# SeekStorm/SeekStorm

Measured on AMD Instinct MI355X. Metric: queries/sec (BM25 3-term OR top-10), higher is better.
Workload: dtype f32 sums of 16-bit posting weight codes (BM25); f32 MFMA (vector); 1 GPU; C2: 10M synthetic docs, 3-term OR BM25 top-10, one shard per GPU; host pointers in, answers on the host; queries_per_call=1000, k=10

## Files before the change

### seekstorm_amd/csrc/bm25_probe.hip

```cpp
#include <cstdlib>
#include <type_traits>

#include "bm25_probe_body.h"


__global__ void __launch_bounds__(256) bm_partmax_kernel(const bm_vquery* __restrict__ qs, const float* __restrict__ submax, uint32_t n_sub,
                                                         uint32_t n_terms, uint32_t nq, uint32_t P, float* __restrict__ pmax) {
  const uint32_t a = (blockIdx.x * blockDim.x + threadIdx.x) >> 6;
  const int lane = threadIdx.x & 63;
  if (a >= nq * P) return;
  const uint32_t qi = a % nq, part = a / nq;
  const bm_vquery* __restrict__ Q = qs + qi;
  const uint32_t s_begin = (uint32_t)(((u64)n_sub * part) / P), s_end = (uint32_t)(((u64)n_sub * (part + 1)) / P);
  for (uint32_t t = 0; t < 4u; t++) {
    const uint32_t term = t < Q->n_terms ? Q->term[t] : n_terms;
    float m = 0.f;
    for (uint32_t sb = s_begin + (uint32_t)lane; sb < s_end; sb += 64u) m = fmaxf(m, submax[(size_t)term * n_sub + sb]);
#pragma unroll
    for (int o = 32; o > 0; o >>= 1) m = fmaxf(m, __shfl_xor(m, o));
    if (lane == 0) pmax[((size_t)qi * P + part) * 4u + t] = m;
  }
}

__global__ void __launch_bounds__(256) bm_qbound_kernel(const bm_vquery* __restrict__ qs, const float* __restrict__ submax, uint32_t n_sub,
                                                        uint32_t nq, float* __restrict__ qbound) {
  const uint32_t q = blockIdx.y, sb = blockIdx.x * blockDim.x + threadIdx.x;
  if (q >= nq || sb >= n_sub) return;
  const bm_vquery* __restrict__ Q = qs + q;
  float b = 0.f;
  for (uint32_t t = 0; t < Q->n_terms; t++) b = fmaf(Q->idf[t], submax[(size_t)Q->term[t] * n_sub + sb], b);
  qbound[(size_t)q * n_sub + sb] = b * 1.00001f;
}

constexpr int PB_STAGED_G = 4;
#ifndef PB_STAGED_WAVES
#define PB_STAGED_WAVES 2
#endif
#ifndef PB_STAGED_MIN_WAVES
#define PB_STAGED_MIN_WAVES 6
#endif
static_assert(PB_STAGED_WAVES == 1 || PB_STAGED_WAVES == 2 || PB_STAGED_WAVES == 4 || PB_STAGED_WAVES == 8, "PB_STAGED_WAVES");
static_assert(PB_STAGED_MIN_WAVES == 6 || PB_STAGED_MIN_WAVES == 8, "PB_STAGED_MIN_WAVES");
static_assert((32 / PB_STAGED_WAVES) * (PB_STAGED_WAVES * pb_wave_lds(4, PB_STAGED_G)) <= 160 * 1024,
              "8 waves per SIMD of the staged kernel (32 / PB_STAGED_WAVES workgroups) must fit a CU's LDS");
constexpr int pb_staged_min_waves(int NT, int KPL, bool FILT, bool SKIP, bool HIST) {
  return KPL == 1 && !(NT == 4 && !FILT && !SKIP && HIST) ? PB_STAGED_MIN_WAVES : 6;
}
template <int NT, int KPL, bool FILT, bool SKIP, bool HIST>
__global__ void __launch_bounds__(PB_STAGED_WAVES * 64, pb_staged_min_waves(NT, KPL, FILT, SKIP, HIST)) bm25_probe_kernel(
    const uint32_t* __restrict__ post, const unsigned long long* __restrict__ term_base, const uint32_t* __restrict__ sub_off,
    const uint2* __restrict__ probe, const uint32_t* __restrict__ probe_z,
    const uint32_t* __restrict__ probe_row, const float* __restrict__ umax, const float* __restrict__ pmax, const float* __restrict__ qbound,
    const bm_vquery* __restrict__ qs, unsigned long long* __restrict__ part_keys, unsigned long long* __restrict__ total,
    uint32_t* tau, uint32_t* hist, const uint32_t* __restrict__ del, uint32_t del_words, uint32_t n_sub, uint32_t n_terms,
    uint32_t nq, uint32_t P, uint32_t k, uint32_t count) {
  extern __shared__ __attribute__((aligned(16))) char smem[];
  if ((uint32_t)(uintptr_t)(__attribute__((address_space(3))) char*)smem != 0u) __builtin_trap();
  const int tid = threadIdx.x, lane = tid & 63;
  const int w = __builtin_amdgcn_readfirstlane(tid >> 6);

  const uint32_t a = blockIdx.x * PB_STAGED_WAVES + w;
  if (a >= nq * P) return;
  const uint32_t qi = a % nq, part = a / nq;
  const BmTop<KPL> T = pb_wave<NT, KPL, FILT, SKIP, false, PB_STAGED_G, false, false, HIST>(
      post, term_base, sub_off, probe, probe_z, probe_row, umax, pmax, qbound, PbQueryMem{qs + qi}, tau, del, del_words, n_sub, n_terms, P, k, count, qi, part,
      w, lane, 0.f, nullptr, 1u, HIST ? hist + (size_t)qi * BM_HIST_B : nullptr);

  u64* out = part_keys + ((size_t)qi * P + part) * (64 * KPL);
#pragma unroll
  for (int r = 0; r < KPL; r++) out[r * 64 + lane] = T.keys[r];
  if (lane == 0 && T.matched) atomicAdd(&total[qi], T.matched);
}

template <int NT, int KPL, bool FILT, bool SKIP, bool HIST>
static int launch_probe(const BmParams& p, const uint2* probe, const uint32_t* probe_z, const uint32_t* probe_row, const float* umax,
                        const float* pmax, const float* qbound, hipStream_t st) {
  const uint32_t A = p.nq * p.P;
#if PB_STATS
  void* stats = nullptr;
  SS_HIP(hipGetSymbolAddress(&stats, HIP_SYMBOL(pb_stats_dev)));
  SS_HIP(hipMemsetAsync(stats, 0, sizeof(pb_stats_dev), st));
#endif
  bm25_probe_kernel<NT, KPL, FILT, SKIP, HIST><<<(A + PB_STAGED_WAVES - 1) / PB_STAGED_WAVES, PB_STAGED_WAVES * 64,
                                                 PB_STAGED_WAVES * pb_wave_lds(NT, PB_STAGED_G), st>>>(
      p.post, p.term_base, p.sub_off, probe, probe_z, probe_row, umax, pmax, qbound, p.q, p.part_keys, p.total, p.tau, p.hist, p.del, p.del_words, p.n_sub, p.n_terms, p.nq, p.P, p.k,
      p.count);
  return SS_OK;
}

constexpr int CNT_WAVES = 4, CNT_UNROLL = 4;
__global__ void __launch_bounds__(CNT_WAVES * 64) bm25_union_count_kernel(
    const uint2* __restrict__ probe, const uint32_t* __restrict__ probe_row, const bm_vquery* __restrict__ qs,
    unsigned long long* __restrict__ total, const uint32_t* __restrict__ del, uint32_t del_words, uint32_t n_sub, uint32_t nq,
    uint32_t P, uint32_t all_queries, unsigned long long* __restrict__ match_bits ) {
  const int lane = threadIdx.x & 63;
  const uint32_t a = blockIdx.x * CNT_WAVES + (threadIdx.x >> 6);
  if (a >= nq * P) return;
  const uint32_t qi = a % nq, part = a / nq;
  const bm_vquery* __restrict__ Q = qs + qi;
  const uint32_t np = Q->n_terms, n_not = bm_q_nnot(Q->op);
  const bool is_and = Q->and_target != 0u;
  if (!all_queries && (is_and || np < 2)) return;
  const uint32_t n_groups = n_sub * (BM_SUB / 64);
  if (match_bits) match_bits += (size_t)qi * n_groups;
  const uint32_t g_begin = (uint32_t)(((u64)n_groups * part) / P), g_end = (uint32_t)(((u64)n_groups * (part + 1)) / P);
  constexpr int CNT_FAST = 8;
  const uint2* rows[CNT_FAST];
#pragma unroll
  for (int t = 0; t < CNT_FAST; t++)
    rows[t] = probe + (size_t)probe_row[(uint32_t)t < np + n_not ? Q->term[t] : Q->term[0]] * n_groups;
  uint32_t cnt = 0;
  for (uint32_t g0 = g_begin; g0 < g_end; g0 += 64u * CNT_UNROLL) {
    u64 acc[CNT_UNROLL], cur[CNT_UNROLL], neg[CNT_UNROLL];
#pragma unroll
    for (int u = 0; u < CNT_UNROLL; u++) { acc[u] = is_and ? ~0ull : 0ull; cur[u] = 0ull; neg[u] = 0ull; }
    if (!is_and) {
#pragma unroll
      for (int t = 0; t < CNT_FAST; t++) {
        if ((uint32_t)t >= np + n_not) break;
#pragma unroll
        for (int u = 0; u < CNT_UNROLL; u++) {
          const uint32_t g = g0 + 64u * u + lane;
          uint2 r = make_uint2(0u, 0u);
          if (g < g_end) r = rows[t][g];
          const u64 b = ((u64)r.y << 32) | r.x;
          if ((uint32_t)t < np) acc[u] |= b; else neg[u] |= b;
        }
      }
      for (uint32_t t = CNT_FAST; t < np + n_not; t++) {
        const uint2* __restrict__ row = probe + (size_t)probe_row[Q->term[t]] * n_groups;
#pragma unroll
        for (int u = 0; u < CNT_UNROLL; u++) {
          const uint32_t g = g0 + 64u * u + lane;
          uint2 r = make_uint2(0u, 0u);
          if (g < g_end) r = row[g];
          const u64 b = ((u64)r.y << 32) | r.x;
          if (t < np) acc[u] |= b; else neg[u] |= b;
        }
      }
    } else {
      uint32_t grp = Q->group[0], seen = np ? 1u : 0u;
      for (uint32_t t = 0; t < np + n_not; t++) {
        const uint2* __restrict__ row = probe + (size_t)probe_row[Q->term[t]] * n_groups;
        const uint32_t gt = Q->group[t];
        if (t < np && gt != grp) {
#pragma unroll
          for (int u = 0; u < CNT_UNROLL; u++) { acc[u] &= cur[u]; cur[u] = 0ull; }
          grp = gt;
          seen++;
        }
        const bool matches = t >= np || Q->and_val[t] != 0;
#pragma unroll
        for (int u = 0; u < CNT_UNROLL; u++) {
          const uint32_t g = g0 + 64u * u + lane;
          uint2 r = make_uint2(0u, 0u);
          if (g < g_end) r = row[g];
          const u64 b = ((u64)r.y << 32) | r.x;
          if (t < np) { if (matches) cur[u] |= b; } else neg[u] |= b;
        }
      }
#pragma unroll
      for (int u = 0; u < CNT_UNROLL; u++) acc[u] = seen == Q->n_groups ? acc[u] & cur[u] : 0ull;
    }
    if (del) {
#pragma unroll
      for (int u = 0; u < CNT_UNROLL; u++) {
        const uint32_t g = g0 + 64u * u + lane;
        if (g < g_end && 2u * g + 1u < del_words) {
          const uint2 r = ((const uint2*)del)[g];
          neg[u] |= ((u64)r.y << 32) | r.x;
        } else if (g < g_end && 2u * g < del_words) {
          neg[u] |= (u64)del[2u * g];
        }
      }
    }
#pragma unroll
    for (int u = 0; u < CNT_UNROLL; u++) cnt += (uint32_t)__popcll(acc[u] & ~neg[u]);
    if (match_bits) {
#pragma unroll
      for (int u = 0; u < CNT_UNROLL; u++) {
        const uint32_t g = g0 + 64u * u + lane;
        if (g < g_end) match_bits[g] = acc[u] & ~neg[u];
      }
    }
  }
  for (int o = 32; o > 0; o >>= 1) cnt += __shfl_xor(cnt, o);
  if (lane == 0 && cnt) atomicAdd(&total[qi], (unsigned long long)cnt);
}

int ssi_bm25_launch_union_count(const BmParams& p, const uint2* probe, const uint32_t* probe_row, bool all_queries, hipStream_t st,
                                unsigned long long* match_bits) {
  const uint32_t n_groups = p.n_sub * (BM_SUB / 64);
  uint32_t P = std::max<uint32_t>(1u, std::min<uint32_t>((2u * 8192u + p.nq - 1) / p.nq, (n_groups + 1023u) / 1024u));
  const uint32_t A = p.nq * P;
  bm25_union_count_kernel<<<(A + CNT_WAVES - 1) / CNT_WAVES, CNT_WAVES * 64, 0, st>>>(probe, probe_row, p.q, p.total, p.del, p.del_words,
                                                                                     p.n_sub, p.nq, P, all_queries ? 1u : 0u, match_bits);
  return SS_OK;
}

int ssi_bm25_launch_probe(const BmParams& p, const uint2* probe, const uint32_t* probe_z, const uint32_t* probe_row, const float* umax,
                          const float* submax, float* pmax_ws, uint32_t nt_max, int KPL, bool any_not, hipStream_t st) {
  const float* pmax = nullptr;
  const float* qbound = nullptr;
  if (submax && pmax_ws) {
    const uint32_t A = p.nq * p.P;
    bm_partmax_kernel<<<(A + 3) / 4, 256, 0, st>>>(p.q, submax, p.n_sub, p.n_terms, p.nq, p.P, pmax_ws);
    float* qb = pmax_ws + (size_t)A * 4u;
    bm_qbound_kernel<<<dim3((p.n_sub + 255) / 256, p.nq), 256, 0, st>>>(p.q, submax, p.n_sub, p.nq, qb);
    pmax = pmax_ws;
    qbound = qb;
  }
  if (!probe || !probe_z || !probe_row || !umax || nt_max == 0 || nt_max > 4 || (KPL != 1 && KPL != 2)) return SS_ENOTSUP;
  const int NT = nt_max <= 2 ? 2 : (int)nt_max;
  const bool filt = any_not || p.del != nullptr;
#define SS_L(NT_, KPL_, F_, S_) \
  (p.hist ? launch_probe<NT_, KPL_, F_, S_, true>(p, probe, probe_z, probe_row, umax, pmax, qbound, st) \
          : launch_probe<NT_, KPL_, F_, S_, false>(p, probe, probe_z, probe_row, umax, pmax, qbound, st))
#define SS_P(NT_, KPL_)                                                                          \
  if (NT == NT_ && KPL == KPL_)                                                                  \
    return qbound ? (filt ? SS_L(NT_, KPL_, true, true) : SS_L(NT_, KPL_, false, true))          \
                  : (filt ? SS_L(NT_, KPL_, true, false) : SS_L(NT_, KPL_, false, false));
  SS_P(2, 1) SS_P(3, 1) SS_P(4, 1) SS_P(2, 2) SS_P(3, 2) SS_P(4, 2)
#undef SS_P
#undef SS_L
  return SS_ENOTSUP;
}

#if PB_STATS
extern "C" int ssi_dbg_pb_stats(unsigned long long* out4) {
  SS_HIP(hipDeviceSynchronize());
  SS_HIP(hipMemcpyFromSymbol(out4, HIP_SYMBOL(pb_stats_dev), 4 * sizeof(unsigned long long)));
  return SS_OK;
}
#endif
```

### seekstorm_amd/csrc/bm25_probe_body.h

```cpp
#pragma once
#include <cstdlib>
#include <type_traits>

#include "bm25_dev.h"
#include "bm25_hist.h"

constexpr int PB_WAVES = 8;
#ifndef PB_TWO_PHASE
#define PB_TWO_PHASE 1
#endif
constexpr bool pb_two_phase(int NT) { return PB_TWO_PHASE != 0 && NT >= 3; }
constexpr int pb_qcap(int NT, int G) { return 64 * G + (pb_two_phase(NT) ? 128 : 64); }
constexpr int pb_wave_lds(int NT, int G) { return pb_qcap(NT, G) * 12; }
#ifndef PB_STATS
#define PB_STATS 0
#endif
#if PB_STATS
static __device__ unsigned long long pb_stats_dev[4];
#endif
#ifndef PB_HIST_READ
#define PB_HIST_READ 1
#endif

__device__ __forceinline__ float pb_weight(uint32_t p) { return bm_weight(p); }
__device__ __forceinline__ uint32_t pb_uniform(uint32_t v) { return (uint32_t)__builtin_amdgcn_readfirstlane((int)v); }
template <typename T>
__device__ __forceinline__ const T* pb_uniform(const T* p) {
  const unsigned long long v = (unsigned long long)(uintptr_t)p;
  return (const T*)(uintptr_t)(((unsigned long long)pb_uniform((uint32_t)(v >> 32)) << 32) | pb_uniform((uint32_t)v));
}

struct PbQueryMem {
  const bm_vquery* __restrict__ q;
  __device__ __forceinline__ uint32_t n_terms() const { return q->n_terms; }
  __device__ __forceinline__ uint32_t op() const { return q->op; }
  __device__ __forceinline__ uint32_t term(int t) const { return q->term[t]; }
  __device__ __forceinline__ float idf(int t) const { return q->idf[t]; }
  __device__ __forceinline__ uint32_t not_term(uint32_t nt, uint32_t j) const { return q->term[nt + j]; }
};
template <int NT>
struct PbQueryRegs {
  uint32_t nt_, op_, term_[NT], not_[4];
  float idf_[NT];
  __device__ __forceinline__ uint32_t n_terms() const { return nt_; }
  __device__ __forceinline__ uint32_t op() const { return op_; }
  __device__ __forceinline__ uint32_t term(int t) const { return term_[t]; }
  __device__ __forceinline__ float idf(int t) const { return idf_[t]; }
  __device__ __forceinline__ uint32_t not_term(uint32_t, uint32_t j) const { return j == 0u ? not_[0] : j == 1u ? not_[1] : j == 2u ? not_[2] : not_[3]; }
};

__device__ __attribute__((noinline)) void pb_publish_kth_best(unsigned long long* bests, uint32_t stride, uint32_t P, uint32_t part, uint32_t k, u64 best, uint32_t* tau_q) {
  const int lane = __lane_id();
  if (lane == 0) __hip_atomic_store(bests + (size_t)part * stride, best, __ATOMIC_RELAXED, __HIP_MEMORY_SCOPE_AGENT);
  const uint32_t step = (P + 255u) / 256u;
  u64 m = 0ull;
  for (uint32_t p_ = (uint32_t)lane * step; p_ < P; p_ += 64u * step) {
    const u64 x = p_ == part ? best : __hip_atomic_load(bests + (size_t)p_ * stride, __ATOMIC_RELAXED, __HIP_MEMORY_SCOPE_AGENT);
    m = x > m ? x : m;
  }
  m = wave_sort_desc(m, lane);
  const u64 kth = rdlane64(m, (int)k - 1);
  if (kth && lane == 0) bm_publish_tau(tau_q, __uint_as_float((uint32_t)(kth >> 32)));
}

__device__ __attribute__((noinline)) void pb_publish_kth_best2(unsigned long long* bests, uint32_t P, uint32_t part, uint32_t k, u64 best, u64 second, uint32_t* tau_q) {
  const int lane = __lane_id();
  if (lane == 0) {
    __hip_atomic_store(bests + (size_t)part * 2u, best, __ATOMIC_RELAXED, __HIP_MEMORY_SCOPE_AGENT);
    __hip_atomic_store(bests + (size_t)part * 2u + 1u, second, __ATOMIC_RELAXED, __HIP_MEMORY_SCOPE_AGENT);
  }
  const uint32_t step = (P + 255u) / 256u;
  u64 m0 = 0ull, m1 = 0ull;
  for (uint32_t p_ = (uint32_t)lane * step; p_ < P; p_ += 64u * step) {
    const u64 x0 = p_ == part ? best : __hip_atomic_load(bests + (size_t)p_ * 2u, __ATOMIC_RELAXED, __HIP_MEMORY_SCOPE_AGENT);
    u64 x1 = p_ == part ? second : __hip_atomic_load(bests + (size_t)p_ * 2u + 1u, __ATOMIC_RELAXED, __HIP_MEMORY_SCOPE_AGENT);
    if (x1 >= x0) x1 = 0ull;
    if (x0 > m0) { m1 = m0 > x1 ? m0 : x1; m0 = x0; }
    else if (x0 > m1) m1 = x0;
  }
  u64 kk[2] = {0ull, 0ull};
  (void)topk_merge64<2>(kk, m0, 128u, lane);
  (void)topk_merge64<2>(kk, m1, 128u, lane);
  const u64 kth = k <= 64u ? rdlane64(kk[0], (int)k - 1) : rdlane64(kk[1], (int)k - 65);
  if (kth && lane == 0) bm_publish_tau(tau_q, __uint_as_float((uint32_t)(kth >> 32)));
}

__device__ __attribute__((noinline)) void pb_publish_hist(uint32_t* hist_q, uint32_t* tau_q, u64 key, uint32_t k, bool read) {
  const uint32_t lo_bits = tau_q[BM_TAU_HIST_LO], shift = tau_q[BM_TAU_HIST_SHIFT];
  if (key) {
    const uint32_t b = bm_hist_bucket((uint32_t)(key >> 32), lo_bits, shift);
    if (b != BM_HIST_NONE) (void)__hip_atomic_fetch_add(hist_q + b, 1u, __ATOMIC_RELAXED, __HIP_MEMORY_SCOPE_AGENT);
  }
  if (!read) return;
  const int lane = __lane_id();
  uint32_t c = __hip_atomic_load(hist_q + lane, __ATOMIC_RELAXED, __HIP_MEMORY_SCOPE_AGENT);
#pragma unroll
  for (int o = 1; o < 64; o <<= 1) {
    const uint32_t x = __shfl_down(c, o);
    if (lane + o < 64) c += x;
  }
  const u64 m = __ballot(c >= k);
  if (m && lane == 0) bm_publish_tau(tau_q, __uint_as_float(bm_hist_edge(63u - (uint32_t)__builtin_clzll(m), lo_bits, shift)));
}

template <int NT, int KPL, bool FILT, bool SKIP, bool SEEDED, int G, bool KTHB, bool EXT = false, bool HIST = false, typename QV>
__device__ __forceinline__ BmTop<KPL> pb_wave(
    const uint32_t* __restrict__ post, const unsigned long long* __restrict__ term_base, const uint32_t* __restrict__ sub_off,
    const uint2* __restrict__ probe, const uint32_t* __restrict__ probe_z,
    const uint32_t* __restrict__ probe_row, const float* __restrict__ umax, const float* __restrict__ pmax, const float* __restrict__ qbound,
    const QV Q, uint32_t* tau, const uint32_t* __restrict__ del, uint32_t del_words, uint32_t n_sub, uint32_t n_terms,
    uint32_t P, uint32_t k, uint32_t count, const uint32_t qi, const uint32_t part, const int w, const int lane, const float thr0 = 0.f,
    unsigned long long* bests = nullptr , const uint32_t bests_stride = 1u,
    uint32_t* hist_q = nullptr ) {
  if (FILT && (del_words >> 31)) { del_words &= 0x7FFFFFFFu; del += (size_t)qi * del_words; }
    const uint32_t nt = Q.n_terms(), n_not = FILT ? bm_q_nnot(Q.op()) : 0u;
  const bool is_and = (bm_q_op(Q.op()) == SS_OP_INTERSECTION) && nt > 1;
  const uint32_t row_len = n_sub + 1;

  const uint32_t* tptr[NT];
  const uint32_t* rowp[NT];
  const uint2* prow[NT];
  const uint32_t* zrow[NT];
  float idf[NT], U[NT];
  uint32_t qpos[NT];
  unsigned long long size[NT];
  const uint32_t s_begin = (uint32_t)(((u64)n_sub * part) / P);
  const uint32_t s_end = (uint32_t)(((u64)n_sub * (part + 1)) / P);
#pragma unroll
  for (int t = 0; t < NT; t++) {
    const bool have = (uint32_t)t < nt;
    const uint32_t term = have ? Q.term(t) : n_terms;
    idf[t] = have ? Q.idf(t) : 0.f;
    U[t] = idf[t] * (pmax ? pmax[((size_t)qi * P + part) * 4u + t] : umax[term]);
    qpos[t] = t;
    tptr[t] = post + term_base[term] * 4ull;
    rowp[t] = sub_off + (size_t)term * row_len;
    prow[t] = probe + (size_t)probe_row[term] * n_sub * (BM_SUB / 64);
    zrow[t] = probe_z + (size_t)probe_row[term] * n_sub * (BM_SUB / 64);
    size[t] = have ? term_base[term + 1] - term_base[term] : ~0ull;
  }
  auto cswap = [&](int x, int y) {
    const bool sw = is_and ? (size[y] < size[x]) : (U[y] > U[x]);
    if (sw) {
      { auto t_ = tptr[x]; tptr[x] = tptr[y]; tptr[y] = t_; }
      { auto t_ = rowp[x]; rowp[x] = rowp[y]; rowp[y] = t_; }
      { auto t_ = prow[x]; prow[x] = prow[y]; prow[y] = t_; }
      { auto t_ = zrow[x]; zrow[x] = zrow[y]; zrow[y] = t_; }
      { float t_ = idf[x]; idf[x] = idf[y]; idf[y] = t_; }
      { float t_ = U[x]; U[x] = U[y]; U[y] = t_; }
      { uint32_t t_ = qpos[x]; qpos[x] = qpos[y]; qpos[y] = t_; }
      { auto t_ = size[x]; size[x] = size[y]; size[y] = t_; }
    }
  };
  if (NT == 2) { cswap(0, 1); }
  if (NT == 3) { cswap(0, 1); cswap(1, 2); cswap(0, 1); }
  if (NT == 4) { cswap(0, 1); cswap(2, 3); cswap(0, 2); cswap(1, 3); cswap(1, 2); }
  float SU[NT + 1];
  SU[NT] = 0.f;
#pragma unroll
  for (int j = NT - 1; j >= 0; j--) SU[j] = SU[j + 1] + U[j];

  BmTop<KPL> T;
#pragma unroll
  for (int r = 0; r < KPL; r++) T.keys[r] = 0ull;
  T.worst = 0ull;
  T.wsc = -1.0f;
  T.matched = 0;
  uint32_t* tau_q = tau + (size_t)qi * BM_TAU_STRIDE;
  u64 last_best = 0ull, last_second = 0ull;
  const int lane4 = lane * 4;

  auto combine = [&](const float (&wv)[NT], uint32_t pres) -> float {
    float score = 0.f;
#pragma unroll
    for (uint32_t qp = 0; qp < (uint32_t)NT; qp++) {
#pragma unroll
      for (int t = 0; t < NT; t++)
        if (qpos[t] == qp && (pres >> t) & 1u) score = fmaf(idf[t], wv[t], score);
    }
    return score;
  };

#if PB_STATS
  uint32_t st_hist = 0u;
#endif
  auto offer = [&](bool cand, float score, uint32_t doc) {
    if (__ballot(cand)) {
      const u64 key = cand ? (((u64)__float_as_uint(score) << 32) | (u64)(0xFFFFFFFFu - doc)) : 0ull;
      const u64 key2 = key > T.worst ? key : 0ull;
      if (__ballot(key2 != 0ull)) {
        T = bm_offer_lane_keys<KPL>(T, key2, k, tau_q);
        if (HIST && hist_q && !is_and) {
          const bool read = PB_HIST_READ == 0 || T.worst != 0ull;
          pb_publish_hist(hist_q, tau_q, key2, k, read);
#if PB_STATS
          st_hist += read ? 1u : 0u;
#endif
        }
        if (KTHB && KPL == 1) {
          const u64 best = rdlane64(T.keys[0], 0);
          if (bests && !is_and && best != last_best) { last_best = best; pb_publish_kth_best(bests, bests_stride, P, part, k, best, tau_q); }
        }
        if (KTHB && KPL == 2) {
          const u64 best = rdlane64(T.keys[0], 0), second = rdlane64(T.keys[0], 1);
          if (bests && !is_and && (best != last_best || second != last_second)) {
            last_best = best; last_second = second;
            pb_publish_kth_best2(bests, P, part, k, best, second, tau_q);
          }
        }
      }
    }
  };
  auto is_deleted = [&](bool lanes, uint32_t doc) -> bool {
    uint32_t wd = 0u;
    if (lanes && (doc >> 5) < del_words) wd = del[doc >> 5];
    return (wd >> (doc & 31u)) & 1u;
  };
  auto in_not_list = [&](bool lanes, uint32_t doc) -> bool {
    bool found = false;
    for (uint32_t j = 0; j < n_not; j++) {
      const uint32_t term = Q.not_term(nt, j);
      uint2 r = make_uint2(0u, 0u);
      if (lanes) r = probe[((size_t)probe_row[term] * n_sub + (doc >> BM_SUB_LOG2)) * (BM_SUB / 64) + ((doc & (BM_SUB - 1)) >> 6)];
      const u64 bits = ((u64)r.y << 32) | r.x;
      found = found || ((bits >> (doc & 63u)) & 1ull);
    }
    return found;
  };
  auto cur_thr = [&]() -> float {
    const float own = SEEDED ? fmaxf(T.wsc, thr0) : T.wsc;
    return fmaxf(own, __uint_as_float(__hip_atomic_load(tau_q, __ATOMIC_RELAXED, __HIP_MEMORY_SCOPE_AGENT)));
  };

  constexpr uint32_t QCAP = pb_qcap(NT, G);
  const uint32_t q_doc = (uint32_t)w * (uint32_t)pb_wave_lds(NT, G), q_w0 = q_doc + QCAP * 4u, q_pos = q_w0 + QCAP * 4u;
  uint32_t qn = 0;
  constexpr bool TWO = pb_two_phase(NT);
  uint32_t q2n = 0;
#if PB_STATS
  uint32_t st_push = 0u, st_pass = 0u, st_apost = 0u;
#endif

  auto stream = [&](auto Jc, auto Sc) {
    constexpr int J = decltype(Jc)::value;
    constexpr bool SINGLE = decltype(Sc)::value;
    constexpr int A = J == 0 ? 1 : 0;
    if (J > 0 && !is_and && k && SU[J] < cur_thr() * 0.99999f) return;
    const uint32_t x_begin = pb_uniform(rowp[J][s_begin]) * 4u, x_end = pb_uniform(rowp[J][s_end]) * 4u;
    if (x_begin == x_end) return;
    if (J == 0 && !is_and && k && !(count && nt == 1) && SU[0] < cur_thr() * 0.99999f) return;

    auto fetch = [&](uint32_t n) {
      const float thr = cur_thr();
      bool alive = (uint32_t)lane < n;
      const uint32_t eb = (QCAP - 1u - (q2n - n + (uint32_t)lane)) * 4u;
      const uint32_t doc = alive ? lds_ld32(q_doc + eb) : 0u;
      const uint32_t rks = alive ? lds_ld32(q_pos + eb) : 0xFFFFFFFFu;
      float wv[NT];
#pragma unroll
      for (int t = 0; t < NT; t++) wv[t] = 0.f;
      wv[J] = alive ? lds_ldf(q_w0 + eb) : 0.f;
      uint32_t pres = 1u << J;
      const uint32_t gidx = (doc >> BM_SUB_LOG2) * (uint32_t)(BM_SUB / 64) + ((doc & (BM_SUB - 1)) >> 6);
      uint32_t zt[NT];
#pragma unroll
      for (int t = 0; t < NT; t++) {
        zt[t] = 0u;
        if (t == J || (uint32_t)t >= nt) continue;
        zt[t] = zrow[t][((rks >> (8 * t)) & 0xFFu) != 0xFFu ? gidx : 0u];
      }
#pragma unroll
      for (int t = 0; t < NT; t++) {
        if (t == J || (uint32_t)t >= nt) continue;
        const uint32_t rk = (rks >> (8 * t)) & 0xFFu;
        if (rk != 0xFFu) {
          wv[t] = pb_weight(tptr[t][zt[t] + rk]);
          pres |= 1u << t;
        }
      }
#if PB_STATS
      st_apost += (uint32_t)__popcll(__ballot(((rks >> (8 * A)) & 0xFFu) != 0xFFu));
#endif
      if (FILT && del && __ballot(alive)) alive = alive && !is_deleted(alive, doc);
      if (FILT && n_not && !(count && is_and) && k) alive = alive && combine(wv, pres) >= thr;
      if (FILT && n_not && __ballot(alive)) alive = alive && !in_not_list(alive, doc);
      if (__ballot(alive)) {
        if (count && is_and) T.matched += __popcll(__ballot(alive));
        if (k) {
          const float score = combine(wv, pres);
          offer(alive && score >= thr && score > 0.f, score, doc);
        }
      }
      q2n -= n;
    };

    auto sift = [&](uint32_t n) {
      const float thr = cur_thr();
      bool alive = (uint32_t)lane < n;
      const uint32_t qb = (qn - n + (uint32_t)lane) * 4u;
      const uint32_t doc = alive ? lds_ld32(q_doc + qb) : 0u;
      const uint32_t pos = alive ? lds_ld32(q_pos + qb) : 0xFFFFFFFFu;
      const float w0 = alive ? lds_ldf(q_w0 + qb) : 0.f;
      const uint32_t d = doc & (BM_SUB - 1);
      const uint32_t gidx = (doc >> BM_SUB_LOG2) * (uint32_t)(BM_SUB / 64) + (d >> 6);
      uint2 rb[NT];
#pragma unroll
      for (int t = 0; t < NT; t++) {
        rb[t] = make_uint2(0u, 0u);
        if (t == J || t == A || (uint32_t)t >= nt) continue;
        rb[t] = prow[t][alive ? gidx : 0u];
      }
      const bool hit_a = pos != 0xFFFFFFFFu;
      float ub = idf[J] * w0 + (hit_a ? U[A] : 0.f);
      uint32_t rks = 0xFFFFFFFFu ^ ((hit_a ? (pos ^ 0xFFu) : 0u) << (8 * A));
      bool hit[NT];
#pragma unroll
      for (int t = 0; t < NT; t++) {
        hit[t] = false;
        if (t == J || t == A || (uint32_t)t >= nt) continue;
        const u64 bits = ((u64)rb[t].y << 32) | rb[t].x;
        hit[t] = alive && ((bits >> (d & 63u)) & 1ull);
        if (is_and) alive = hit[t];
        else if (t < J && hit[t]) { alive = false; }
        const uint32_t rk = (uint32_t)__popcll(bits & ((1ull << (d & 63u)) - 1ull));
        if (hit[t]) { rks ^= (rk ^ 0xFFu) << (8 * t); ub += U[t]; }
      }
      if (!is_and && k) alive = alive && ub >= thr * 0.99999f;
      const u64 m = __ballot(alive);
      if (m) {
        if (alive) {
          const uint32_t at = (QCAP - 1u - (q2n + (uint32_t)__popcll(m & ((1ull << lane) - 1ull)))) * 4u;
          lds_st32(q_doc + at, doc);
          lds_stf(q_w0 + at, w0);
          lds_st32(q_pos + at, rks);
        }
        q2n += (uint32_t)__popcll(m);
      }
#if PB_STATS
      st_pass += (uint32_t)__popcll(m);
#endif
      qn -= n;
      while (q2n >= 64u) fetch(64u);
    };

    auto drain = [&](uint32_t n) {
      const float thr = cur_thr();
      bool alive = (uint32_t)lane < n;
      const uint32_t qb = (qn - n + (uint32_t)lane) * 4u;
      const uint32_t doc = alive ? lds_ld32(q_doc + qb) : 0u;
      const uint32_t pos = alive ? lds_ld32(q_pos + qb) : 0xFFFFFFFFu;
      const uint32_t tile = doc >> BM_SUB_LOG2, d = doc & (BM_SUB - 1);
      float wv[NT];
#pragma unroll
      for (int t = 0; t < NT; t++) wv[t] = 0.f;
      wv[J] = alive ? lds_ldf(q_w0 + qb) : 0.f;
      uint32_t pres = 1u << J;
      float known = idf[J] * wv[J];
      const uint32_t gidx = tile * (uint32_t)(BM_SUB / 64) + (d >> 6);
      const bool hit_a = alive && pos != 0xFFFFFFFFu;
      const uint32_t za = zrow[A][hit_a ? gidx : 0u];
      uint2 rb[NT];
#pragma unroll
      for (int t = 0; t < NT; t++) {
        rb[t] = make_uint2(0u, 0u);
        if (t == J || t == A || (uint32_t)t >= nt) continue;
        rb[t] = prow[t][alive ? gidx : 0u];
      }
      uint32_t pa = 0u;
      if (hit_a) pa = tptr[A][za + pos];
      bool hit[NT];
      uint32_t zt[NT], rk[NT];
#pragma unroll
      for (int t = 0; t < NT; t++) {
        hit[t] = false; zt[t] = 0u; rk[t] = 0u;
        if (t == J || t == A || (uint32_t)t >= nt) continue;
        const u64 bits = ((u64)rb[t].y << 32) | rb[t].x;
        hit[t] = alive && ((bits >> (d & 63u)) & 1ull);
        if (is_and) alive = hit[t];
        else if (t < J && hit[t]) { alive = false; }
        rk[t] = (uint32_t)__popcll(bits & ((1ull << (d & 63u)) - 1ull));
      }
#pragma unroll
      for (int t = 0; t < NT; t++) {
        hit[t] = hit[t] && alive;
        if (t == J || t == A || (uint32_t)t >= nt) continue;
        zt[t] = zrow[t][hit[t] ? gidx : 0u];
      }
      if (hit_a) {
        wv[A] = pb_weight(pa);
        pres |= 1u << A;
        known += idf[A] * wv[A];
      }
      float rest = SU[0] - U[J] - ((uint32_t)A < nt ? U[A] : 0.f);
      if (!is_and && k) alive = alive && (known + rest) >= thr * 0.99999f;
#if PB_STATS
      st_pass += (uint32_t)__popcll(__ballot(alive));
      st_apost += (uint32_t)__popcll(__ballot(hit_a));
#endif
#pragma unroll
      for (int t = 0; t < NT; t++) {
        if (t == J || t == A || (uint32_t)t >= nt) continue;
        if (hit[t] && alive) {
          const uint32_t pt = tptr[t][zt[t] + rk[t]];
          wv[t] = pb_weight(pt);
          pres |= 1u << t;
        }
      }
      if (FILT && del && __ballot(alive)) alive = alive && !is_deleted(alive, doc);
      if (FILT && n_not && !(count && is_and) && k) alive = alive && combine(wv, pres) >= thr;
      if (FILT && n_not && __ballot(alive)) alive = alive && !in_not_list(alive, doc);
      if (__ballot(alive)) {
        if (count && is_and) T.matched += __popcll(__ballot(alive));
        if (k) {
          const float score = combine(wv, pres);
          offer(alive && score >= thr && score > 0.f, score, doc);
        }
      }
      qn -= n;
    };

    __amdgpu_buffer_rsrc_t rs = __builtin_amdgcn_make_buffer_rsrc((void*)pb_uniform(tptr[J]), 0, (int)(x_end * 4u), BM_RSRC_FLAGS);
    uint32_t blk0 = s_begin;
    uint32_t vb = rowp[J][min(blk0 + (uint32_t)lane, s_end)] * 4u;
    const bool skip_blocks = SKIP && k != 0 && !count;
    const float* __restrict__ qbrow = SKIP ? qbound + (size_t)qi * n_sub : nullptr;
    uint32_t vqb = 0u;
    if constexpr (SKIP) { if (skip_blocks) vqb = __float_as_uint(qbrow[min(blk0 + (uint32_t)lane, s_end - 1u)]); }
    auto bnd = [&](uint32_t s) -> uint32_t {
      return __builtin_amdgcn_readlane(vb, s - blk0);
    };
    uint32_t s_cur = s_begin;
    uint32_t pn[G];
#pragma unroll
    for (int g = 0; g < G; g++) pn[g] = __builtin_amdgcn_raw_buffer_load_b32(rs, lane4 + g * 256, (int)(x_begin * 4u), 0);
    constexpr bool THR_FIRST = J > 0 || EXT || SKIP;
    for (uint32_t x = x_begin; x < x_end; x += 64u * G) {
      float thr = 0.f;
      if constexpr (THR_FIRST) thr = __uint_as_float(pb_uniform(__float_as_uint(cur_thr())));
      if (!is_and && k && (J > 0 || (EXT && !(count && nt == 1))) && SU[J] < thr * 0.99999f) break;
      if constexpr (SKIP) if (skip_blocks) {
        bool moved = false;
        const float thr_s = thr * 0.99999f;
        for (;;) {
          if (s_cur + 1u - blk0 >= 64u) {
            blk0 = s_cur;
            vb = rowp[J][min(blk0 + (uint32_t)lane, s_end)] * 4u;
            vqb = __float_as_uint(qbrow[min(blk0 + (uint32_t)lane, s_end - 1u)]);
          }
          if (s_cur + 1u > s_end) break;
          const uint32_t b1 = bnd(s_cur + 1u);
          if (b1 <= x) { s_cur++; continue; }
          if (__uint_as_float(__builtin_amdgcn_readlane(vqb, s_cur - blk0)) >= thr_s) break;
          x = b1;
          s_cur++;
          moved = true;
          if (x >= x_end) break;
        }
        if (moved) {
          if (x >= x_end) break;
#pragma unroll
          for (int g = 0; g < G; g++) pn[g] = __builtin_amdgcn_raw_buffer_load_b32(rs, lane4 + g * 256, (int)(x * 4u), 0);
        }
      }
      uint32_t pg[G], tile[G];
#pragma unroll
      for (int g = 0; g < G; g++) {
        pg[g] = pn[g];
        tile[g] = s_cur;
      }
      const uint32_t x_hi = min(x + 64u * G, x_end);
      for (;;) {
        if (s_cur + 1u - blk0 >= 64u) {
          blk0 = s_cur;
          vb = rowp[J][min(blk0 + (uint32_t)lane, s_end)] * 4u;
          if constexpr (SKIP) { if (skip_blocks) vqb = __float_as_uint(qbrow[min(blk0 + (uint32_t)lane, s_end - 1u)]); }
        }
        if (s_cur + 1u > s_end) break;
        const uint32_t b = bnd(s_cur + 1u);
        if (b >= x_hi) break;
        s_cur++;
#pragma unroll
        for (int g = 0; g < G; g++) tile[g] += (x + 64u * g + (uint32_t)lane) >= b ? 1u : 0u;
      }
      uint32_t dg[G];
      bool alive[G];
      float w0[G];
      uint2 rec[G];
      if constexpr (!THR_FIRST) thr = cur_thr();
#pragma unroll
      for (int g = 0; g < G; g++) {
        alive[g] = pg[g] != 0u;
        dg[g] = bm_doc_field(pg[g]) - 1u;
        if (!SINGLE) rec[g] = prow[A][alive[g] ? tile[g] * (uint32_t)(BM_SUB / 64) + (dg[g] >> 6) : 0u];
      }
#pragma unroll
      for (int g = 0; g < G; g++) pn[g] = __builtin_amdgcn_raw_buffer_load_b32(rs, lane4 + g * 256, (int)(x_hi * 4u), 0);
#pragma unroll
      for (int g = 0; g < G; g++) w0[g] = alive[g] ? pb_weight(pg[g]) : 0.f;
      if constexpr (SINGLE) {
#pragma unroll
        for (int g = 0; g < G; g++) {
          if (__ballot(alive[g]) == 0ull) continue;
          const uint32_t doc1 = (tile[g] << BM_SUB_LOG2) + dg[g];
          if (FILT && del && count) alive[g] = alive[g] && !is_deleted(alive[g], doc1);
          if (FILT && n_not && count) alive[g] = alive[g] && !in_not_list(alive[g], doc1);
          if (count) T.matched += __popcll(__ballot(alive[g]));
          if (k) {
            const float score = fmaf(idf[J], w0[g], 0.f);
            bool cand = alive[g] && score >= thr && score > 0.f;
            if (FILT && del && !count && __ballot(cand)) cand = cand && !is_deleted(cand, doc1);
            if (FILT && n_not && !count && __ballot(cand)) cand = cand && !in_not_list(cand, doc1);
            offer(cand, score, doc1);
          }
        }
      } else {
        const float rest0 = SU[0] - U[J];
#pragma unroll
        for (int g = 0; g < G; g++)
          if (!is_and && k) alive[g] = alive[g] && (idf[J] * w0[g] + rest0) >= thr * 0.99999f;
#pragma unroll
        for (int g = 0; g < G; g++) {
          const u64 bits = ((u64)rec[g].y << 32) | rec[g].x;
          bool hit = alive[g] && ((bits >> (dg[g] & 63u)) & 1ull);
          uint32_t pos = 0xFFFFFFFFu;
          if (is_and) alive[g] = hit;
          else if (A < J && hit) { alive[g] = false; hit = false; }
          else if (!hit && k) alive[g] = alive[g] && (idf[J] * w0[g] + rest0 - U[A]) >= thr * 0.99999f;
          if (hit) pos = (uint32_t)__popcll(bits & ((1ull << (dg[g] & 63u)) - 1ull));
          const u64 m = __ballot(alive[g]);
          if (m) {
            if (alive[g]) {
              const uint32_t at = qn + (uint32_t)__popcll(m & ((1ull << lane) - 1ull));
              lds_st32(q_doc + at * 4u, (tile[g] << BM_SUB_LOG2) + dg[g]);
              lds_stf(q_w0 + at * 4u, w0[g]);
              lds_st32(q_pos + at * 4u, pos);
            }
            qn += (uint32_t)__popcll(m);
#if PB_STATS
            st_push += (uint32_t)__popcll(m);
#endif
          }
        }
        if constexpr (TWO) { while (qn >= 64u) sift(64u); }
        else { while (qn >= 64u) drain(64u); }
      }
    }
    if constexpr (SINGLE) {
    } else if constexpr (TWO) {
      if (qn) sift(qn);
      if (q2n) fetch(q2n);
    } else {
      if (qn) drain(qn);
    }
  };
  if (nt == 1) stream(std::integral_constant<int, 0>{}, std::true_type{});
  else if (k || is_and) stream(std::integral_constant<int, 0>{}, std::false_type{});
  if (!is_and && k) {
    if (NT > 1 && nt > 1) stream(std::integral_constant<int, (NT > 1 ? 1 : 0)>{}, std::false_type{});
    if (NT > 2 && nt > 2) stream(std::integral_constant<int, (NT > 2 ? 2 : 0)>{}, std::false_type{});
    if (NT > 3 && nt > 3) stream(std::integral_constant<int, (NT > 3 ? 3 : 0)>{}, std::false_type{});
  }

#if PB_STATS
  if (lane == 0) {
    atomicAdd(&pb_stats_dev[0], (unsigned long long)st_push);
    atomicAdd(&pb_stats_dev[1], (unsigned long long)st_pass);
    atomicAdd(&pb_stats_dev[2], (unsigned long long)st_apost);
    atomicAdd(&pb_stats_dev[3], (unsigned long long)st_hist);
  }
#endif
  return T;
}
```

Measured before the change: 2.110 million queries/s.

## Software-pipeline first-term posting walk with one-tile-ahead probe gather

Adds an AHEAD variant of the first-term (J==0) posting scan in the staged probe kernel. It computes sub-block tiles and gathers the probe bitmap records for the next tile, and prefetches the posting words after that, before processing the current tile. The aim is to hide global-load latency of probe rows behind the dense scoring and LDS queue work. This costs extra registers for the double-buffered state, so the min-waves launch bound drops to 6 for those instantiations. It applies only to specific NT/KPL/FILT/HIST combinations without SKIP.

```diff
diff --git a/seekstorm_amd/csrc/bm25_probe.hip b/seekstorm_amd/csrc/bm25_probe.hip
--- a/seekstorm_amd/csrc/bm25_probe.hip
+++ b/seekstorm_amd/csrc/bm25_probe.hip
@@ -43,8 +43,14 @@
 static_assert(PB_STAGED_MIN_WAVES == 6 || PB_STAGED_MIN_WAVES == 8, "PB_STAGED_MIN_WAVES");
 static_assert((32 / PB_STAGED_WAVES) * (PB_STAGED_WAVES * pb_wave_lds(4, PB_STAGED_G)) <= 160 * 1024,
               "8 waves per SIMD of the staged kernel (32 / PB_STAGED_WAVES workgroups) must fit a CU's LDS");
+#ifndef PB_AHEAD
+#define PB_AHEAD 1
+#endif
+constexpr bool pb_staged_ahead(int NT, int KPL, bool FILT, bool SKIP, bool HIST) {
+  return PB_AHEAD != 0 && !SKIP && (KPL == 1 ? !(NT == 4 && FILT && !HIST) : (NT == 3 && FILT && HIST));
+}
 constexpr int pb_staged_min_waves(int NT, int KPL, bool FILT, bool SKIP, bool HIST) {
-  return KPL == 1 && !(NT == 4 && !FILT && !SKIP && HIST) ? PB_STAGED_MIN_WAVES : 6;
+  return KPL == 1 && !(NT == 4 && !FILT && !SKIP && HIST) && !pb_staged_ahead(NT, KPL, FILT, SKIP, HIST) ? PB_STAGED_MIN_WAVES : 6;
 }
 template <int NT, int KPL, bool FILT, bool SKIP, bool HIST>
 __global__ void __launch_bounds__(PB_STAGED_WAVES * 64, pb_staged_min_waves(NT, KPL, FILT, SKIP, HIST)) bm25_probe_kernel(
@@ -62,7 +68,7 @@
   const uint32_t a = blockIdx.x * PB_STAGED_WAVES + w;
   if (a >= nq * P) return;
   const uint32_t qi = a % nq, part = a / nq;
-  const BmTop<KPL> T = pb_wave<NT, KPL, FILT, SKIP, false, PB_STAGED_G, false, false, HIST>(
+  const BmTop<KPL> T = pb_wave<NT, KPL, FILT, SKIP, false, PB_STAGED_G, false, false, HIST, pb_staged_ahead(NT, KPL, FILT, SKIP, HIST)>(
       post, term_base, sub_off, probe, probe_z, probe_row, umax, pmax, qbound, PbQueryMem{qs + qi}, tau, del, del_words, n_sub, n_terms, P, k, count, qi, part,
       w, lane, 0.f, nullptr, 1u, HIST ? hist + (size_t)qi * BM_HIST_B : nullptr);
 
diff --git a/seekstorm_amd/csrc/bm25_probe_body.h b/seekstorm_amd/csrc/bm25_probe_body.h
--- a/seekstorm_amd/csrc/bm25_probe_body.h
+++ b/seekstorm_amd/csrc/bm25_probe_body.h
@@ -103,7 +103,7 @@
   if (m && lane == 0) bm_publish_tau(tau_q, __uint_as_float(bm_hist_edge(63u - (uint32_t)__builtin_clzll(m), lo_bits, shift)));
 }
 
-template <int NT, int KPL, bool FILT, bool SKIP, bool SEEDED, int G, bool KTHB, bool EXT = false, bool HIST = false, typename QV>
+template <int NT, int KPL, bool FILT, bool SKIP, bool SEEDED, int G, bool KTHB, bool EXT = false, bool HIST = false, bool AHEAD = false, typename QV>
 __device__ __forceinline__ BmTop<KPL> pb_wave(
     const uint32_t* __restrict__ post, const unsigned long long* __restrict__ term_base, const uint32_t* __restrict__ sub_off,
     const uint2* __restrict__ probe, const uint32_t* __restrict__ probe_z,
@@ -434,6 +434,96 @@
 #pragma unroll
     for (int g = 0; g < G; g++) pn[g] = __builtin_amdgcn_raw_buffer_load_b32(rs, lane4 + g * 256, (int)(x_begin * 4u), 0);
     constexpr bool THR_FIRST = J > 0 || EXT || SKIP;
+    if constexpr (AHEAD && J == 0 && !SKIP && !EXT && !SINGLE) {
+      auto walk = [&](const uint32_t x, const uint32_t x_hi, uint32_t (&tile)[G]) {
+#pragma unroll
+        for (int g = 0; g < G; g++) tile[g] = s_cur;
+        for (;;) {
+          if (s_cur + 1u - blk0 >= 64u) {
+            blk0 = s_cur;
+            vb = rowp[J][min(blk0 + (uint32_t)lane, s_end)] * 4u;
+          }
+          if (s_cur + 1u > s_end) break;
+          const uint32_t b = bnd(s_cur + 1u);
+          if (b >= x_hi) break;
+          s_cur++;
+#pragma unroll
+          for (int g = 0; g < G; g++) tile[g] += (x + 64u * g + (uint32_t)lane) >= b ? 1u : 0u;
+        }
+      };
+      auto gather = [&](const uint32_t (&pg)[G], const uint32_t (&tile)[G], uint2 (&rec)[G]) {
+#pragma unroll
+        for (int g = 0; g < G; g++) rec[g] = prow[A][pg[g] != 0u ? tile[g] * (uint32_t)(BM_SUB / 64) + ((bm_doc_field(pg[g]) - 1u) >> 6) : 0u];
+      };
+      auto prefetch = [&](const uint32_t at) {
+#pragma unroll
+        for (int g = 0; g < G; g++) pn[g] = __builtin_amdgcn_raw_buffer_load_b32(rs, lane4 + g * 256, (int)(at * 4u), 0);
+      };
+      auto dense = [&](const uint32_t (&pg)[G], const uint32_t (&tile)[G], const uint2 (&rec)[G], const float thr) {
+        uint32_t dg[G];
+        bool alive[G];
+        float w0[G];
+#pragma unroll
+        for (int g = 0; g < G; g++) {
+          alive[g] = pg[g] != 0u;
+          dg[g] = bm_doc_field(pg[g]) - 1u;
+        }
+#pragma unroll
+        for (int g = 0; g < G; g++) w0[g] = alive[g] ? pb_weight(pg[g]) : 0.f;
+        const float rest0 = SU[0] - U[J];
+#pragma unroll
+        for (int g = 0; g < G; g++)
+          if (!is_and && k) alive[g] = alive[g] && (idf[J] * w0[g] + rest0) >= thr * 0.99999f;
+#pragma unroll
+        for (int g = 0; g < G; g++) {
+          const u64 bits = ((u64)rec[g].y << 32) | rec[g].x;
+          bool hit = alive[g] && ((bits >> (dg[g] & 63u)) & 1ull);
+          uint32_t pos = 0xFFFFFFFFu;
+          if (is_and) alive[g] = hit;
+          else if (A < J && hit) { alive[g] = false; hit = false; }
+          else if (!hit && k) alive[g] = alive[g] && (idf[J] * w0[g] + rest0 - U[A]) >= thr * 0.99999f;
+          if (hit) pos = (uint32_t)__popcll(bits & ((1ull << (dg[g] & 63u)) - 1ull));
+          const u64 m = __ballot(alive[g]);
+          if (m) {
+            if (alive[g]) {
+              const uint32_t at = qn + (uint32_t)__popcll(m & ((1ull << lane) - 1ull));
+              lds_st32(q_doc + at * 4u, (tile[g] << BM_SUB_LOG2) + dg[g]);
+              lds_stf(q_w0 + at * 4u, w0[g]);
+              lds_st32(q_pos + at * 4u, pos);
+            }
+            qn += (uint32_t)__popcll(m);
+#if PB_STATS
+            st_push += (uint32_t)__popcll(m);
+#endif
+          }
+        }
+        if constexpr (TWO) { while (qn >= 64u) sift(64u); }
+        else { while (qn >= 64u) drain(64u); }
+      };
+      uint32_t pg[G], tile[G];
+      uint2 rec[G];
+      uint32_t x_hi = min(x_begin + 64u * G, x_end);
+#pragma unroll
+      for (int g = 0; g < G; g++) pg[g] = pn[g];
+      walk(x_begin, x_hi, tile);
+      gather(pg, tile, rec);
+      prefetch(x_hi);
+      for (uint32_t x = x_begin; x < x_end; x += 64u * G) {
+        uint32_t pg1[G], tile1[G];
+        uint2 rec1[G];
+#pragma unroll
+        for (int g = 0; g < G; g++) pg1[g] = pn[g];
+        const uint32_t x_hi1 = min(x_hi + 64u * G, x_end);
+        walk(x_hi, x_hi1, tile1);
+        const float thr = cur_thr();
+        gather(pg1, tile1, rec1);
+        prefetch(x_hi1);
+        dense(pg, tile, rec, thr);
+#pragma unroll
+        for (int g = 0; g < G; g++) { pg[g] = pg1[g]; tile[g] = tile1[g]; rec[g] = rec1[g]; }
+        x_hi = x_hi1;
+      }
+    } else
     for (uint32_t x = x_begin; x < x_end; x += 64u * G) {
       float thr = 0.f;
       if constexpr (THR_FIRST) thr = __uint_as_float(pb_uniform(__float_as_uint(cur_thr())));
```

Result: slower. 2.088 million queries/s (-1.0%).
